# zyhbili/Dual-Space-NeRF

Hardware: AMD Instinct MI355X
Metric: rendered rays/sec (64 samples/ray), 512x512 frame (higher is better)
Workload: dtype split-f16x3 (3 x v_mfma_f32_32x32x16_f16 on hi/lo fp16 operand halves, f32 accumulate: f32-equivalent accuracy - parity bars of the tests: 1e-4 absolute on RGB / acc / weights against the reference; sigma 1e-4 absolute where |sigma| <= 100 and 4e-6 RELATIVE to max|sigma| above (this checkpoint: |sig

## Files before the change

### dual-space-nerf_amd/csrc/dsn_field16.hip

```cpp
#include "dsn_common.h"
#include "dsn_kernels.h"

typedef float f32x16 __attribute__((ext_vector_type(16)));
typedef _Float16 half8 __attribute__((ext_vector_type(8)));
#define MFMA16(a, b, c) __builtin_amdgcn_mfma_f32_32x32x16_f16((a), (b), (c), 0, 0, 0)

#if !defined(DSN_EXPERIMENTS) && (defined(F16_ABL) || defined(F16_SABL) || defined(F16_TIMING) || defined(F16_TRAIN_ABL))
#error "F16_ABL / F16_SABL / F16_TIMING are experiment switches (wrong results / debug counters): build with -DDSN_EXPERIMENTS"
#endif
#ifndef F16_SINCOS_OCML
#define F16_SINCOS_OCML 0
#endif
#ifndef F16_FENCE
#define F16_FENCE 0
#endif
#ifndef F16_SGB
#define F16_SGB 1
#endif
#ifndef F16_SGB_VALU
#define F16_SGB_VALU 4
#endif
#ifndef F16_SGB_DS
#define F16_SGB_DS 0
#endif
// ... 52 lines not shown
    char* ring;
    unsigned ring_off;
    int wave;
    int nchunk = F16_NCHUNK;
    bool spread = F16_DMA_SPREAD != 0;
    half8 h0, l0, h1, l1;
};

#ifndef F16_POS_OFFS
#define F16_POS_OFFS 0
#endif
__device__ __forceinline__ void w16_stage(const W16& w, int c) {
    const char* src = w.g + (size_t)c * 32768;
    const unsigned dst = w.ring_off + (c & 1) * 32768 + w.wave * 8192 + 4096;
#if F16_POS_OFFS
    asm volatile("s_mov_b32 m0, %1\n\ts_nop 0\n\t"
                 "global_load_lds_dwordx4 %0, off\n\tglobal_load_lds_dwordx4 %0, off offset:1024\n\t"
                 "global_load_lds_dwordx4 %0, off offset:2048\n\tglobal_load_lds_dwordx4 %0, off offset:3072"
                 : : "v"(src - 4096), "s"(dst - 4096) : "memory", "m0");
    asm volatile("s_mov_b32 m0, %1\n\ts_nop 0\n\t"
                 "global_load_lds_dwordx4 %0, off\n\tglobal_load_lds_dwordx4 %0, off offset:1024\n\t"
                 "global_load_lds_dwordx4 %0, off offset:2048\n\tglobal_load_lds_dwordx4 %0, off offset:3072"
                 : : "v"(src), "s"(dst) : "memory", "m0");
    return;
#endif
    asm volatile("s_mov_b32 m0, %1\n\ts_nop 0\n\t"
                 "global_load_lds_dwordx4 %0, off offset:-4096\n\tglobal_load_lds_dwordx4 %0, off offset:-3072\n\t"
                 "global_load_lds_dwordx4 %0, off offset:-2048\n\tglobal_load_lds_dwordx4 %0, off offset:-1024\n\t"
                 "global_load_lds_dwordx4 %0, off\n\tglobal_load_lds_dwordx4 %0, off offset:1024\n\t"
                 "global_load_lds_dwordx4 %0, off offset:2048\n\tglobal_load_lds_dwordx4 %0, off offset:3072"
                 : : "v"(src), "s"(dst) : "memory", "m0");
}
template <int I>
__device__ __forceinline__ void w16_stage_part(const W16& w, int c) {
    const char* src = w.g + (size_t)c * 32768;
    const unsigned dst = w.ring_off + (c & 1) * 32768 + w.wave * 8192 + 4096;
#if F16_POS_OFFS
    {
        const int back = I < 2 ? 4096 : 0;
        asm volatile("s_mov_b32 m0, %1\n\ts_nop 0\n\t"
                     "global_load_lds_dwordx4 %0, off offset:%2\n\tglobal_load_lds_dwordx4 %0, off offset:%3"
                     : : "v"(src - back), "s"(dst - back), "n"(2048 * (I & 1)), "n"(2048 * (I & 1) + 1024) : "memory", "m0");
        return;
    }
#endif
    asm volatile("s_mov_b32 m0, %1\n\ts_nop 0\n\t"
                 "global_load_lds_dwordx4 %0, off offset:%2\n\tglobal_load_lds_dwordx4 %0, off offset:%3"
                 : : "v"(src), "s"(dst), "n"(-4096 + 2048 * I), "n"(-3072 + 2048 * I) : "memory", "m0");
}
__device__ __forceinline__ void w16_boundary(const W16& w, int b) {
#if !(F16_ABL & 2)
    asm volatile("s_waitcnt vmcnt(0)" ::: "memory");
#endif
#if !(F16_ABL & 1)
    __syncthreads();
#endif
    const int c = b / F16_CHUNK;
#if !(F16_ABL & 4)
    if (!w.spread && c + 1 < w.nchunk) w16_stage(w, c + 1);
#endif
}
__device__ __forceinline__ void w16_read(const W16& w, int b, int lane, half8& h0, half8& l0, half8& h1, half8& l1) {
    const char* s = w.ring + ((b >> 3) & 1) * 32768 + (b & 7) * 1024 + lane * 16;
    h0 = *reinterpret_cast<const half8*>(s);
    l0 = *reinterpret_cast<const half8*>(s + 8192);
    h1 = *reinterpret_cast<const half8*>(s + 16384);
    l1 = *reinterpret_cast<const half8*>(s + 24576);
}
__device__ __forceinline__ void w16_begin_issue(W16& w, int first_blk) { w16_stage(w, first_blk / F16_CHUNK); }
__device__ __forceinline__ void w16_begin_wait(W16& w, int lane, int first_blk) {
    w16_boundary(w, first_blk);
#if !(F16_ABL & 4)
    if (w.spread && first_blk / F16_CHUNK + 1 < w.nchunk) w16_stage_part<0>(w, first_blk / F16_CHUNK + 1);
#endif
    w16_read(w, first_blk, lane, w.h0, w.l0, w.h1, w.l1);
}
__device__ __forceinline__ void w16_begin(W16& w, int lane, int first_blk) {
    w16_begin_issue(w, first_blk);
    w16_begin_wait(w, lane, first_blk);
}

struct NoHook { __device__ __forceinline__ void operator()(int) const {} };

template <int KB, bool XLS, class Hook = NoHook>
__device__ __forceinline__ void dense16(W16& w, int& blk, int lane, const half8 (&xh)[KB][2], const half8 (&xl)[KB][2],
                                        f32x16& accM, f32x16& accC, Hook&& hook = NoHook()) {
#pragma unroll
    for (int kb = 0; kb < KB; ++kb) {
#if F16_PREFETCH
        half8 n0 = w.h0, m0 = w.l0, n1 = w.h1, m1 = w.l1;
        if (blk + 1 < DSN_STREAM_BLOCKS) {
            if (((blk + 1) & (F16_CHUNK - 1)) == 0) w16_boundary(w, blk + 1);
#if !(F16_ABL & 4)
            if (w.spread) {
                const int pos = (blk + 1) & (F16_CHUNK - 1), cn = (blk + 1) / F16_CHUNK + 1;
                if (cn < w.nchunk) {
                    if (pos == 0) w16_stage_part<0>(w, cn);
                    if (pos == 1) w16_stage_part<1>(w, cn);
                    if (pos == 2) w16_stage_part<2>(w, cn);
                    if (pos == 3) w16_stage_part<3>(w, cn);
                }
            }
#endif
            w16_read(w, blk + 1, lane, n0, m0, n1, m1);
        }
#else
        if (blk > 0) {
            if ((blk & (F16_CHUNK - 1)) == 0) w16_boundary(w, blk);
            w16_read(w, blk, lane, w.h0, w.l0, w.h1, w.l1);
        }
#endif
        if (XLS) {
            accM = MFMA16(w.h0, xh[kb][0], accM);
            accC = MFMA16(w.h0, xl[kb][0], accC);
            accC = MFMA16(w.l0, xh[kb][0], accC);
            accM = MFMA16(w.h1, xh[kb][1], accM);
            accC = MFMA16(w.h1, xl[kb][1], accC);
            accC = MFMA16(w.l1, xh[kb][1], accC);
        } else {
            accM = MFMA16(w.h0, xh[kb][0], accM);
            accC = MFMA16(w.l0, xh[kb][0], accC);
            accM = MFMA16(w.h0, xl[kb][0], accM);
            accC = MFMA16(w.h1, xh[kb][1], accC);
            accM = MFMA16(w.l1, xh[kb][1], accM);
            accC = MFMA16(w.h1, xl[kb][1], accC);
        }
#if !(F16_ABL & 8)
        hook(kb);
#endif
#if F16_PREFETCH
        w.h0 = n0; w.l0 = m0; w.h1 = n1; w.l1 = m1;
#endif
        ++blk;
#if F16_SGB
#if F16_SGB_DS == 2
        __builtin_amdgcn_sched_group_barrier(0x100, 4, 0);
#endif
#pragma unroll
        for (int i = 0; i < 6; ++i) {
            __builtin_amdgcn_sched_group_barrier(0x008, 1, 0);
#if F16_SGB_DS == 1
            if (i < 4) __builtin_amdgcn_sched_group_barrier(0x100, 1, 0);
#endif
            __builtin_amdgcn_sched_group_barrier(0x002, F16_SGB_VALU, 0);
        }
        __builtin_amdgcn_sched_barrier(0);
#endif
#if F16_FENCE
        __builtin_amdgcn_sched_barrier(0);
#endif
    }
}

__device__ __forceinline__ f32x16 rows16(const float* __restrict__ v, int m, int half) {
    f32x16 o;
#pragma unroll
    for (int q = 0; q < 4; ++q) {
        const float4 t = *reinterpret_cast<const float4*>(v + 32 * m + 8 * q + 4 * half);
        o[4 * q + 0] = t.x; o[4 * q + 1] = t.y; o[4 * q + 2] = t.z; o[4 * q + 3] = t.w;
    }
    return o;
}
__device__ __forceinline__ f32x16 zero16() {
    f32x16 z;
#pragma unroll
    for (int r = 0; r < 16; ++r) z[r] = 0.0f;
    return z;
}
template <bool SCALED>
__device__ __forceinline__ void split16(const f32x16& v, half8 (&h)[2], half8 (&l)[2]) {
#pragma unroll
    for (int r = 0; r < 16; ++r) {
        const _Float16 hi = (_Float16)v[r];
        const float res = fmaf((float)hi, -1.0f, v[r]);
        h[r >> 3][r & 7] = hi;
        l[r >> 3][r & 7] = SCALED ? (_Float16)(res * DSN_LO_SCALE) : (_Float16)res;
    }
}
#define F16_FWD_SCALE 64.0f
#define F16_FWD_INV 0.015625f
__device__ __forceinline__ f32x16 unscale16(const f32x16& m, const f32x16& c) {
    f32x16 v;
#pragma unroll
    for (int r = 0; r < 16; ++r) v[r] = (m[r] + c[r]) * F16_FWD_INV;
    return v;
}
__device__ __forceinline__ f32x16 fold16(const f32x16& m, const f32x16& c) {
    f32x16 v;
#pragma unroll
    for (int r = 0; r < 16; ++r) v[r] = fmaf(c[r], DSN_LO_INV, m[r]);
    return v;
}
__device__ __forceinline__ uint32_t dsn_push_sign(uint32_t word, float v) {
    return __builtin_amdgcn_alignbit(word, __float_as_uint(v), 31);
}
__device__ __forceinline__ uint32_t dsn_active_word(uint32_t signs) { return ~signs & 0xffffu; }
#ifndef F16_KEEP_ASM
#define F16_KEEP_ASM 1
#endif
__device__ __forceinline__ float dsn_keep_active(float v, uint32_t word, int r) {
#if F16_KEEP_ASM
    uint32_t m;
    asm("v_bfe_i32 %0, %1, %2, 1" : "=v"(m) : "v"(word), "s"(15 - r));
    return __uint_as_float(__float_as_uint(v) & m);
#else
    return __uint_as_float(__float_as_uint(v) & (uint32_t)__builtin_amdgcn_sbfe((int)word, 15 - r, 1));
#endif
}
__device__ __forceinline__ uint32_t relu_bits16(f32x16& a) {
    uint32_t s = 0;
#pragma unroll
    for (int r = 0; r < 16; ++r) {
        s = dsn_push_sign(s, a[r]);
        a[r] = fmaxf(a[r], 0.0f);
    }
    return dsn_active_word(s);
}
__device__ __forceinline__ void mask16(f32x16& a, uint32_t m) {
#pragma unroll
    for (int r = 0; r < 16; ++r) a[r] = dsn_keep_active(a[r], m, r);
}

__device__ __forceinline__ void track16(float& ovf, const f32x16& v) {
#pragma unroll
    for (int r = 0; r < 16; r += 2) asm("v_max3_f32 %0, %0, |%1|, |%2|" : "+v"(ovf) : "v"(v[r]), "v"(v[r + 1]));
}
__device__ __forceinline__ float dsn_nan_flag() { return __uint_as_float(0x7fc00000u); }
// ... 60 lines not shown
            const float s0 = vv[0] * DSN_LO_SCALE, s1 = vv[1] * DSN_LO_SCALE;
            asm("v_fma_mixlo_f16 %0, %1, %2, %3 op_sel_hi:[1,0,0]" : "=v"(L) : "v"(H), "s"(k), "v"(s0));
            asm("v_fma_mixhi_f16 %0, %1, %2, %3 op_sel:[1,0,0] op_sel_hi:[1,0,0]" : "+v"(L) : "v"(H), "s"(k), "v"(s1));
        }
        typedef uint32_t u32x4 __attribute__((ext_vector_type(4)));
        u32x4 th = __builtin_bit_cast(u32x4, yh[r >> 3]), tl = __builtin_bit_cast(u32x4, yl[r >> 3]);
        th[(r & 7) >> 1] = H;
        tl[(r & 7) >> 1] = L;
        yh[r >> 3] = __builtin_bit_cast(half8, th);
        yl[r >> 3] = __builtin_bit_cast(half8, tl);
    }
#endif
    if (FWD) asm("v_max3_f32 %0, %0, %1, %2" : "+v"(ovf) : "v"(vv[0]), "v"(vv[1]));
    else asm("v_max3_f32 %0, %0, |%1|, |%2|" : "+v"(ovf) : "v"(vv[0]), "v"(vv[1]));
#if defined(DSN_EXPERIMENTS) && defined(F16_TRAIN_ABL) && (F16_TRAIN_ABL & 256)
    if (ST && kb == 7) {
        float o[16];
#pragma unroll
        for (int r = 0; r < 16; ++r) {
            float v = FWD ? (pM[r] + pC[r]) * F16_FWD_INV : fmaf(pC[r], DSN_LO_INV, pM[r]);
            v = FWD ? fmaxf(v, 0.0f) : dsn_keep_active(v, mword, r);
            o[r] = v * stscale;
        }
        store16_lines_emul(st, o);
        return;
    }
#endif
    if (ST && kb == 7 && st) {
#pragma unroll
        for (int q = 0; q < 4; ++q) {
            float o[4];
#pragma unroll
            for (int e = 0; e < 4; ++e) {
                const int r = 4 * q + e;
                float v = FWD ? (pM[r] + pC[r]) * F16_FWD_INV : fmaf(pC[r], DSN_LO_INV, pM[r]);
                v = FWD ? fmaxf(v, 0.0f) : dsn_keep_active(v, mword, r);
                o[e] = v * stscale;
            }
            *reinterpret_cast<float4*>(st + 8 * q) = make_float4(o[0], o[1], o[2], o[3]);
        }
    }
}
#ifndef F16_NT_STORE
#define F16_NT_STORE 0
#endif
typedef float f32x4 __attribute__((ext_vector_type(4)));
__device__ __forceinline__ void store16(float* st, const f32x16& v, float stscale) {
#if defined(DSN_EXPERIMENTS) && defined(F16_TRAIN_ABL) && (F16_TRAIN_ABL & 4)
    {
        const int lane = threadIdx.x & 63, hf = lane >> 5, i = lane & 3;
        const unsigned long long me = (unsigned long long)(uintptr_t)st;
#pragma unroll
        for (int j = 0; j < 4; ++j) {
            const int src = (lane & ~3) | j;
            const unsigned lo = __shfl((unsigned)me, src), hi = __shfl((unsigned)(me >> 32), src);
            float* pj = reinterpret_cast<float*>((uintptr_t)(((unsigned long long)hi << 32) | lo));
            if (pj) *reinterpret_cast<float4*>(pj - 4 * hf + 16 * hf + 4 * i) =
                make_float4(v[4 * j] * stscale, v[4 * j + 1] * stscale, v[4 * j + 2] * stscale, v[4 * j + 3] * stscale);
        }
        return;
    }
#endif
#if defined(DSN_EXPERIMENTS) && defined(F16_TRAIN_ABL) && (F16_TRAIN_ABL & 256)
    {
        float o[16];
#pragma unroll
        for (int r = 0; r < 16; ++r) o[r] = v[r] * stscale;
        store16_lines_emul(st, o);
        return;
    }
#endif
    if (!st) return;
#pragma unroll
    for (int q = 0; q < 4; ++q) {
#if F16_NT_STORE
        const f32x4 x = {v[4 * q] * stscale, v[4 * q + 1] * stscale, v[4 * q + 2] * stscale, v[4 * q + 3] * stscale};
        __builtin_nontemporal_store(x, reinterpret_cast<f32x4*>(st + 8 * q));
#else
        *reinterpret_cast<float4*>(st + 8 * q) = make_float4(v[4 * q] * stscale, v[4 * q + 1] * stscale, v[4 * q + 2] * stscale, v[4 * q + 3] * stscale);
#endif
    }
}

template <bool ST = false, bool EXTRA = false, bool HEAD = false>
__device__ __forceinline__ void layer16_fwd(W16& w, int& blk, int lane, const float* __restrict__ bias,
                                            const half8 (&xh)[8][2], const half8 (&xl)[8][2], half8 (&yh)[8][2],
                                            half8 (&yl)[8][2], uint32_t (&mk)[4], float& ovf, float* st = nullptr,
                                            const half8 (*s_pe)[F16_THREADS] = nullptr, const float* wden = nullptr, float* sg = nullptr) {
    const int half = lane >> 5;
    const int tid = threadIdx.x;
    f32x16 pM = zero16(), pC = zero16();
#if F16_BIAS_AHEAD
    f32x16 bnext = rows16(bias, 0, half);
#endif
#pragma unroll
    for (int m = 0; m < 8; ++m) {
#if F16_BIAS_AHEAD
        f32x16 aM = bnext, aC = zero16();
        if (m + 1 < 8) bnext = rows16(bias, m + 1, half);
#else
        f32x16 aM = rows16(bias, m, half), aC = zero16();
#endif
        uint32_t bits = 0;
        if (m == 0) dense16<8, false>(w, blk, lane, xh, xl, aM, aC);
        else dense16<8, false>(w, blk, lane, xh, xl, aM, aC, [&](int kb) {
            epi_slice<true, ST, HEAD>(pM, pC, kb, 0u, bits, yh[m - 1], yl[m - 1], ovf, (ST && st) ? st + F16_ST_M(m - 1) : nullptr, 1.0f,
                                      HEAD ? wden + 32 * (m - 1) + 4 * half : nullptr, sg); });
        if (EXTRA) {
            half8 qh[2][2], ql[2][2];
            qh[0][0] = s_pe[0][tid]; qh[0][1] = s_pe[1][tid]; qh[1][0] = s_pe[2][tid]; qh[1][1] = s_pe[3][tid];
            ql[0][0] = s_pe[4][tid]; ql[0][1] = s_pe[5][tid]; ql[1][0] = s_pe[6][tid]; ql[1][1] = s_pe[7][tid];
            dense16<2, false>(w, blk, lane, qh, ql, aM, aC);
        }
        if (m > 0) { if ((m - 1) & 1) mk[(m - 1) >> 1] |= dsn_active_word(bits) << 16; else mk[(m - 1) >> 1] = dsn_active_word(bits); }
        pM = aM; pC = aC;
    }
    {
        uint32_t bits = 0;
#pragma unroll
        for (int kb = 0; kb < 8; ++kb)
            epi_slice<true, ST, HEAD>(pM, pC, kb, 0u, bits, yh[7], yl[7], ovf, (ST && st) ? st + F16_ST_M(7) : nullptr, 1.0f,
                                      HEAD ? wden + 32 * 7 + 4 * half : nullptr, sg);
        mk[3] |= dsn_active_word(bits) << 16;
    }
}
template <bool ST = false>
__device__ __forceinline__ void layer16_bwd(W16& w, int& blk, int lane, const half8 (&xh)[8][2],
                                            const half8 (&xl)[8][2], half8 (&yh)[8][2], half8 (&yl)[8][2],
                                            const uint32_t (&mk)[4], float& ovf, float* st = nullptr, float stscale = F16_GUNSCALE) {
    f32x16 pM = zero16(), pC = zero16();
    uint32_t dummy = 0;
#pragma unroll
    for (int m = 0; m < 8; ++m) {
        f32x16 aM = zero16(), aC = zero16();
        const uint32_t mw = m > 0 ? ((mk[(m - 1) >> 1] >> (16 * ((m - 1) & 1))) & 0xffffu) : 0u;
        if (m == 0) dense16<8, true>(w, blk, lane, xh, xl, aM, aC);
        else dense16<8, true>(w, blk, lane, xh, xl, aM, aC, [&](int kb) { epi_slice<false, ST>(pM, pC, kb, mw, dummy, yh[m - 1], yl[m - 1], ovf, (ST && st) ? st + F16_ST_M(m - 1) : nullptr, stscale); });
        pM = aM; pC = aC;
    }
    const uint32_t mw = (mk[3] >> 16) & 0xffffu;
#pragma unroll
    for (int kb = 0; kb < 8; ++kb) epi_slice<false, ST>(pM, pC, kb, mw, dummy, yh[7], yl[7], ovf, (ST && st) ? st + F16_ST_M(7) : nullptr, stscale);
}

#define F16_FULL 0
#define F16_FWD 1
#define F16_BWD 2
#define F16_TRAIN 3
#define F16_DEN 4
#define F16_FIRST_BWD_BLOCK (OFF_L6T / DSN_BLK)
#define F16_DEN_BLOCKS (F16_FIRST_BWD_BLOCK - 4 * 8)
static_assert(F16_DEN_BLOCKS % F16_CHUNK == 0, "the density-only kernel streams whole chunks");
template <int MODE>
__global__ void __launch_bounds__(F16_THREADS, 1)
k_field16(const float* __restrict__ packed, const DsnFrameState* __restrict__ fs, const float* __restrict__ x_c,
          int64_t N, const int32_t* __restrict__ active_list, const int32_t* __restrict__ active_count,
          float* __restrict__ sigma, float* __restrict__ essence, float* __restrict__ grad,
          uint4* __restrict__ masks, int32_t* __restrict__ pos_list, int32_t* __restrict__ pos_count,
          float* __restrict__ tr_h, float* __restrict__ tr_a, float* __restrict__ tr_rr, int64_t slot_base, int64_t rec_cap,
          const int32_t* __restrict__ sel, int32_t* __restrict__ flag_count) {
    constexpr bool ST = MODE == F16_TRAIN;
    __shared__ __attribute__((aligned(16))) char ring[F16_RING_SLOTS * 4096];
    __shared__ uint32_t s_mask[7][4][F16_THREADS];
    __shared__ __attribute__((aligned(16))) float s_vec[256 + 2304 + 8];
    __shared__ __attribute__((aligned(16))) half8 s_pe[8][F16_THREADS];
    __shared__ int s_app[8];
#ifndef F16_SHARE_SIMD
    DSN_OWN_SIMD();
#endif
    const int tid0 = threadIdx.x;
    const int lane0 = threadIdx.x & 63;
    const int wave = __builtin_amdgcn_readfirstlane(threadIdx.x >> 6);
    int64_t count = (active_list ? (int64_t)(*active_count) : N) - slot_base;
    if (MODE == F16_BWD && count > rec_cap) count = rec_cap;
    const int64_t ntiles = (count + 127) / 128;
    if ((int64_t)blockIdx.x >= ntiles) return;
    for (int i = tid0; i < 256 + 2304 + 8; i += F16_THREADS)
        s_vec[i] = i < 256 ? fs->bias0[i] : (i < 2560 ? packed[OFF_B1 + (i - 256)] : packed[OFF_SCAL + (i - 2560)]);
    for (int i = tid0; i < 256 + (OFF_WDEN - OFF_B1); i += F16_THREADS) s_vec[i] *= F16_FWD_SCALE;
    const float* const v_bias0 = s_vec;
    const float* const v_b1 = s_vec + 256;
    const float* const v_brgb1 = s_vec + 256 + (OFF_BRGB1 - OFF_B1);
    const float* const v_wden = s_vec + 256 + (OFF_WDEN - OFF_B1);
    const float* const v_wrgb3 = s_vec + 256 + (OFF_WRGB3 - OFF_B1);
    const float* const v_scal = s_vec + 2560;
    W16 w;
    w.g = reinterpret_cast<const char*>(packed + OFF16_BASE) + wave * 8192 + 4096 + lane0 * 16;
    w.ring = ring;
    w.ring_off = (unsigned)(uintptr_t)(__attribute__((address_space(3))) char*)ring;
    w.wave = wave;
    if (MODE == F16_FWD) w.nchunk = F16_FIRST_BWD_BLOCK / F16_CHUNK;
    if (MODE == F16_DEN) w.nchunk = F16_DEN_BLOCKS / F16_CHUNK;
    if (MODE == F16_TRAIN) w.spread = false;
    auto tile_point = [&](int64_t t, bool& ok, int64_t& ls) -> int64_t {
        int64_t sl = (t * 4 + wave) * 32 + (lane0 & 31);
        ok = sl < count;
        if (!ok) sl = count - 1;
        ls = sel ? (int64_t)sel[sl] : slot_base + sl;
        return active_list ? (int64_t)active_list[ls] : ls;
    };
    bool valid_n;
    int64_t lslot_n;
    int64_t pt_n = tile_point(blockIdx.x, valid_n, lslot_n);
    float xn[3] = {x_c[3 * pt_n], x_c[3 * pt_n + 1], x_c[3 * pt_n + 2]};
  for (int64_t tile = blockIdx.x; tile < ntiles; tile += gridDim.x) {
    int tid = tid0, lane = lane0;
    asm volatile("" : "+v"(tid), "+v"(lane), "+v"(w.g));
    const int half = lane >> 5;
#if F16_TIMING
    unsigned long long tstamp[6], rstamp[6];
#endif
    F16_STAMP(0);
    w16_begin_issue(w, MODE == F16_BWD ? F16_FIRST_BWD_BLOCK : 0);
#if !F16_NEXT_POINT
    if (tile != (int64_t)blockIdx.x) { pt_n = tile_point(tile, valid_n, lslot_n); xn[0] = x_c[3 * pt_n]; xn[1] = x_c[3 * pt_n + 1]; xn[2] = x_c[3 * pt_n + 2]; }
#endif
    const bool valid = valid_n;
    const int64_t lslot = lslot_n, pt = pt_n;
    const float xa[3] = {xn[0], xn[1], xn[2]};
    const bool more = F16_NEXT_POINT && MODE != F16_TRAIN && tile + gridDim.x < ntiles;
    if (more) pt_n = tile_point(tile + gridDim.x, valid_n, lslot_n);
#define NEXT_POINT() do { if (more) { xn[0] = x_c[3 * pt_n]; xn[1] = x_c[3 * pt_n + 1]; xn[2] = x_c[3 * pt_n + 2]; } } while (0)
    w16_begin_wait(w, lane, MODE == F16_BWD ? F16_FIRST_BWD_BLOCK : 0);
    int blk = MODE == F16_BWD ? F16_FIRST_BWD_BLOCK : 0;
    F16_STAMP(1);

#define MK_STORE(L, mk) { if (MODE != F16_DEN) { s_mask[L][0][tid] = mk[0]; s_mask[L][1][tid] = mk[1]; s_mask[L][2][tid] = mk[2]; s_mask[L][3][tid] = mk[3]; } }
#define MK_LOAD(L, mk) { mk[0] = s_mask[L][0][tid]; mk[1] = s_mask[L][1][tid]; mk[2] = s_mask[L][2][tid]; mk[3] = s_mask[L][3][tid]; }
    uint32_t mk[4];
    half8 ah[8][2], al[8][2], bh[8][2], bl[8][2];
    float ovf = packed[DSN_SPLIT_UNSAFE_FIELD];
    uint4* mrec = masks ? masks + ((size_t)(MODE == F16_BWD ? lslot : pt) * 2 + half) * 7 : nullptr;
    const int64_t tr_ls = N * 256;
#if defined(DSN_EXPERIMENTS) && defined(F16_TRAIN_ABL)
    const int64_t pt_st = (F16_TRAIN_ABL & 8) ? (pt & 4095) : ((F16_TRAIN_ABL & 16) ? (pt & 255) : pt);
    const int64_t sl_st = (tile * 4 + wave) * 32 + (lane & 31);
    const int64_t row_off = (F16_TRAIN_ABL & 32) ? (sl_st >> 5) * 8192 + (sl_st & 31) * 32 : pt_st * 256;
    float* const th = ST && valid && !(F16_TRAIN_ABL & 1) ? tr_h + row_off + 4 * half : nullptr;
    float* const ta = ST && valid && !(F16_TRAIN_ABL & 2) ? tr_a + row_off + 4 * half : nullptr;
#else
    float* const th = ST && valid ? tr_h + pt * 256 + 4 * half : nullptr;
    float* const ta = ST && valid ? tr_a + pt * 256 + 4 * half : nullptr;
#endif

  if (MODE != F16_BWD) {
    half8 ph[2][2], pl[2][2];
    {
        f32x16 pe[2];
#pragma unroll
        for (int t = 0; t < 30; ++t) {
            float s, c;
#if F16_SINCOS_OCML
            sincosf(xa[t % 3] * (float)(1 << (t / 3)), &s, &c);
#else
            dsn_sincos(xa[t % 3] * (float)(1 << (t / 3)), s, c);
#endif
            pe[t >> 4][t & 15] = half ? c : s;
        }
        pe[1][14] = half ? xa[1] : xa[0];
        pe[1][15] = half ? 0.0f : xa[2];
        split16<false>(pe[0], ph[0], pl[0]);
        split16<false>(pe[1], ph[1], pl[1]);
        s_pe[0][tid] = ph[0][0]; s_pe[1][tid] = ph[0][1]; s_pe[2][tid] = ph[1][0]; s_pe[3][tid] = ph[1][1];
        s_pe[4][tid] = pl[0][0]; s_pe[5][tid] = pl[0][1]; s_pe[6][tid] = pl[1][0]; s_pe[7][tid] = pl[1][1];
    }

    F16_STAMP(2);
#pragma unroll
    for (int m = 0; m < 8; ++m) {
        f32x16 aM = rows16(v_bias0, m, half), aC = zero16();
        dense16<2, false>(w, blk, lane, ph, pl, aM, aC);
        f32x16 v = unscale16(aM, aC);
        const uint32_t bits = relu_bits16(v);
        if (m & 1) mk[m >> 1] |= bits << 16; else mk[m >> 1] = bits;
        if (ST) store16(th ? th + 0 * tr_ls + F16_ST_M(m) : nullptr, v, 1.0f);
        track16(ovf, v);
        split16<false>(v, ah[m], al[m]);
    }
    MK_STORE(0, mk)
    layer16_fwd<ST>(w, blk, lane, v_b1 + 0 * 256, ah, al, bh, bl, mk, ovf, th ? th + 1 * tr_ls : nullptr); MK_STORE(1, mk)
    NEXT_POINT();
    layer16_fwd<ST>(w, blk, lane, v_b1 + 1 * 256, bh, bl, ah, al, mk, ovf, th ? th + 2 * tr_ls : nullptr); MK_STORE(2, mk)
    layer16_fwd<ST>(w, blk, lane, v_b1 + 2 * 256, ah, al, bh, bl, mk, ovf, th ? th + 3 * tr_ls : nullptr); MK_STORE(3, mk)
#if F16_PIPE_LATE
    layer16_fwd<ST, true, false>(w, blk, lane, v_b1 + 3 * 256, bh, bl, ah, al, mk, ovf, th ? th + 4 * tr_ls : nullptr, s_pe);
    MK_STORE(4, mk)
    layer16_fwd<ST>(w, blk, lane, v_b1 + 4 * 256, ah, al, bh, bl, mk, ovf, th ? th + 5 * tr_ls : nullptr); MK_STORE(5, mk)
    float sg_part = 0.0f;
    layer16_fwd<ST, false, true>(w, blk, lane, v_b1 + 5 * 256, bh, bl, ah, al, mk, ovf, th ? th + 6 * tr_ls : nullptr, nullptr, v_wden,
                                 &sg_part);
#else
#pragma unroll
    for (int m = 0; m < 8; ++m) {
        f32x16 aM = rows16(v_b1 + 3 * 256, m, half), aC = zero16();
        dense16<8, false>(w, blk, lane, bh, bl, aM, aC);
        {
            half8 qh[2][2], ql[2][2];
            qh[0][0] = s_pe[0][tid]; qh[0][1] = s_pe[1][tid]; qh[1][0] = s_pe[2][tid]; qh[1][1] = s_pe[3][tid];
            ql[0][0] = s_pe[4][tid]; ql[0][1] = s_pe[5][tid]; ql[1][0] = s_pe[6][tid]; ql[1][1] = s_pe[7][tid];
            dense16<2, false>(w, blk, lane, qh, ql, aM, aC);
        }
        f32x16 v = unscale16(aM, aC);
        const uint32_t bits = relu_bits16(v);
        if (m & 1) mk[m >> 1] |= bits << 16; else mk[m >> 1] = bits;
        if (ST) store16(th ? th + 4 * tr_ls + F16_ST_M(m) : nullptr, v, 1.0f);
        track16(ovf, v);
        split16<false>(v, ah[m], al[m]);
    }
    MK_STORE(4, mk)
    layer16_fwd<ST>(w, blk, lane, v_b1 + 4 * 256, ah, al, bh, bl, mk, ovf, th ? th + 5 * tr_ls : nullptr); MK_STORE(5, mk)
    float sg_part = 0.0f;
#pragma unroll
    for (int m = 0; m < 8; ++m) {
        f32x16 aM = rows16(v_b1 + 5 * 256, m, half), aC = zero16();
        dense16<8, false>(w, blk, lane, bh, bl, aM, aC);
        f32x16 v = unscale16(aM, aC);
        const uint32_t bits = relu_bits16(v);
        if (m & 1) mk[m >> 1] |= bits << 16; else mk[m >> 1] = bits;
        if (ST) store16(th ? th + 6 * tr_ls + F16_ST_M(m) : nullptr, v, 1.0f);
        const f32x16 wd = rows16(v_wden, m, half);
#pragma unroll
        for (int r = 0; r < 16; ++r) sg_part = fmaf(wd[r], v[r], sg_part);
        track16(ovf, v);
        split16<false>(v, ah[m], al[m]);
    }
#endif
    F16_STAMP(3);
    sg_part += __shfl_xor(sg_part, 32);
    const float sg = sg_part + v_scal[0];
    const bool flag_fwd = !(fmaxf(ovf, __shfl_xor(ovf, 32)) < F16_RANGE);
    if (valid && half == 0) sigma[pt] = flag_fwd ? dsn_nan_flag() : sg;
    if (MODE != F16_TRAIN && flag_fwd && valid && half == 0 && flag_count) atomicAdd(flag_count, 1);
    ovf = flag_fwd ? __builtin_inff() : 0.0f;
    if (MODE == F16_DEN) { __syncthreads(); continue; }
    bool write_rec = ST && valid;
    if (MODE == F16_FWD) {
        const bool pos = valid && half == 0 && (sg > 0.0f || flag_fwd);
        const unsigned long long bm = __ballot(pos);
        const int cnt = __popcll(bm);
        if (lane == 0) s_app[wave] = cnt;
        __syncthreads();
        if (tid == 0) {
            const int tot = s_app[0] + s_app[1] + s_app[2] + s_app[3];
            s_app[4] = tot ? atomicAdd(pos_count, tot) : 0;
        }
        __syncthreads();
        int base = s_app[4];
        for (int k = 0; k < wave; ++k) base += s_app[k];
        const int my = base + __popcll(bm & ((1ull << lane) - 1ull));
        if (pos) pos_list[my] = (int32_t)pt;
        const int rslot = __shfl(my, lane & 31);
        write_rec = ((bm >> (lane & 31)) & 1ull) != 0 && (int64_t)rslot < rec_cap;
        mrec = masks + ((size_t)rslot * 2 + half) * 7;
    }
    if (MODE == F16_FWD || MODE == F16_TRAIN) {
        MK_STORE(6, mk)
        if (write_rec) {
#pragma unroll
            for (int L = 0; L < 7; ++L)
                mrec[L] = make_uint4(s_mask[L][0][tid], s_mask[L][1][tid], s_mask[L][2][tid], s_mask[L][3][tid]);
        }
    }
    {
        float e0 = 0.f, e1 = 0.f, e2 = 0.f;
#pragma unroll
        for (int m = 0; m < 4; ++m) {
            f32x16 aM = rows16(v_brgb1, m, half), aC = zero16();
            dense16<8, false>(w, blk, lane, ah, al, aM, aC);
            const f32x16 v = unscale16(aM, aC);
            const f32x16 w0 = rows16(v_wrgb3 + 0 * 128, m, half);
            const f32x16 w1 = rows16(v_wrgb3 + 1 * 128, m, half);
            const f32x16 w2 = rows16(v_wrgb3 + 2 * 128, m, half);
            if (ST && valid) {
                f32x16 xr;
#pragma unroll
                for (int r = 0; r < 16; ++r) xr[r] = fmaxf(v[r], 0.0f);
                store16(tr_rr + pt * 128 + 4 * half + 32 * m, xr, 1.0f);
            }
#pragma unroll
            for (int r = 0; r < 16; ++r) {
                const float x = fmaxf(v[r], 0.0f);
                e0 = fmaf(w0[r], x, e0); e1 = fmaf(w1[r], x, e1); e2 = fmaf(w2[r], x, e2);
            }
        }
        e0 += __shfl_xor(e0, 32); e1 += __shfl_xor(e1, 32); e2 += __shfl_xor(e2, 32);
        if (valid && half == 0) {
            essence[3 * pt + 0] = e0 + v_scal[1];
            essence[3 * pt + 1] = e1 + v_scal[2];
            essence[3 * pt + 2] = e2 + v_scal[3];
        }
    }

#if F16_TIMING
    F16_STAMP(4);
    if (MODE == F16_FWD && tid == 0) {
        for (int i = 0; i < 4; ++i) { atomicAdd(&g_f16_timing[i], tstamp[i + 1] - tstamp[i]); atomicAdd(&g_f16_timing[8 + i], rstamp[i + 1] - rstamp[i]); }
        atomicAdd(&g_f16_timing[7], 1ull);
    }
#endif
    if (MODE == F16_FWD) { __syncthreads(); continue; }
  } else {
#pragma unroll
    for (int L = 0; L < 7; ++L) {
        const uint4 q = mrec[L];
        s_mask[L][0][tid] = q.x; s_mask[L][1][tid] = q.y; s_mask[L][2][tid] = q.z; s_mask[L][3][tid] = q.w;
    }
    MK_LOAD(6, mk)
  }

#pragma unroll
    for (int m = 0; m < 8; ++m) {
        f32x16 g = rows16(v_wden, m, half);
#pragma unroll
        for (int r = 0; r < 16; ++r) g[r] *= F16_GSCALE;
        mask16(g, (mk[m >> 1] >> (16 * (m & 1))) & 0xffffu);
        if (ST) store16(ta ? ta + 6 * tr_ls + F16_ST_M(m) : nullptr, g, F16_GUNSCALE);
        split16<true>(g, ah[m], al[m]);
    }
    MK_LOAD(5, mk) layer16_bwd<ST>(w, blk, lane, ah, al, bh, bl, mk, ovf, ta ? ta + 5 * tr_ls : nullptr);
    if (MODE == F16_BWD) NEXT_POINT();
    MK_LOAD(4, mk) layer16_bwd<ST>(w, blk, lane, bh, bl, ah, al, mk, ovf, ta ? ta + 4 * tr_ls : nullptr);
    MK_LOAD(3, mk)
    f32x16 dpe[2];
#pragma unroll
    for (int m = 0; m < 8; ++m) {
        f32x16 aM = zero16(), aC = zero16();
        dense16<8, true>(w, blk, lane, ah, al, aM, aC);
        f32x16 v = fold16(aM, aC);
        mask16(v, (mk[m >> 1] >> (16 * (m & 1))) & 0xffffu);
        if (ST) store16(ta ? ta + 3 * tr_ls + F16_ST_M(m) : nullptr, v, F16_GUNSCALE);
        track16(ovf, v);
        split16<true>(v, bh[m], bl[m]);
    }
#pragma unroll
    for (int b = 0; b < 2; ++b) {
        f32x16 aM = zero16(), aC = zero16();
        dense16<8, true>(w, blk, lane, ah, al, aM, aC);
        dpe[b] = fold16(aM, aC);
    }
    MK_LOAD(2, mk) layer16_bwd<ST>(w, blk, lane, bh, bl, ah, al, mk, ovf, ta ? ta + 2 * tr_ls : nullptr);
    MK_LOAD(1, mk) layer16_bwd<ST>(w, blk, lane, ah, al, bh, bl, mk, ovf, ta ? ta + 1 * tr_ls : nullptr);
    MK_LOAD(0, mk) layer16_bwd<ST>(w, blk, lane, bh, bl, ah, al, mk, ovf, ta ? ta + 0 * tr_ls : nullptr);
#pragma unroll
    for (int b = 0; b < 2; ++b) {
        f32x16 aM = zero16(), aC = zero16();
        dense16<8, true>(w, blk, lane, ah, al, aM, aC);
        const f32x16 v = fold16(aM, aC);
#pragma unroll
        for (int r = 0; r < 16; ++r) dpe[b][r] += v[r];
    }

    {
        float xb[3] = {xa[0], xa[1], xa[2]};
        asm volatile("" : "+v"(xb[0]), "+v"(xb[1]), "+v"(xb[2]));
        float g[3] = {0.f, 0.f, 0.f};
#pragma unroll
        for (int t = 0; t < 30; ++t) {
            const int j = t / 3, a = t % 3;
            float s, c;
#if F16_SINCOS_OCML
            sincosf(xb[a] * (float)(1 << j), &s, &c);
#else
            dsn_sincos(xb[a] * (float)(1 << j), s, c);
#endif
            const float d = dpe[t >> 4][t & 15];
            const float term = (d * (half ? s : c)) * (float)(1 << j);
            g[a] += half ? -term : term;
        }
        const float i30 = dpe[1][14], i31 = dpe[1][15];
        if (half) g[1] += i30; else { g[0] += i30; g[2] += i31; }
        g[0] += __shfl_xor(g[0], 32); g[1] += __shfl_xor(g[1], 32); g[2] += __shfl_xor(g[2], 32);
        if (valid && half == 0) {
            grad[3 * pt] = g[0] * F16_GUNSCALE; grad[3 * pt + 1] = g[1] * F16_GUNSCALE; grad[3 * pt + 2] = g[2] * F16_GUNSCALE;
        }
    }
    const bool flagged = !(fmaxf(ovf, __shfl_xor(ovf, 32)) < F16_RANGE_SCALED);
    if (flagged && valid && half == 0) {
        if (MODE == F16_TRAIN) { if (pos_count) atomicAdd(pos_count, 1); }
        else { sigma[pt] = dsn_nan_flag(); if (flag_count) atomicAdd(flag_count, 1); }
    }
    if (MODE == F16_TRAIN) break;
    __syncthreads();
  }
}

void dsn_launch_field16(const float* packed, const DsnFrameState* fs, const float* x_c, int64_t N,
                        const int32_t* active_list, const int32_t* active_count, float* sigma, float* essence,
                        float* grad, hipStream_t st, int32_t* flag_count) {
    int64_t blocks = (N + 127) / 128;
    if (blocks == 0) return;
    hipLaunchKernelGGL(k_field16<F16_FULL>, dim3((unsigned)std::min<int64_t>(blocks, dsn_cu_count())), dim3(F16_THREADS), 0, st, packed, fs, x_c, N,
                       active_list, active_count, sigma, essence, grad, (uint4*)nullptr, (int32_t*)nullptr,
                       (int32_t*)nullptr, (float*)nullptr, (float*)nullptr, (float*)nullptr, (int64_t)0, (int64_t)0, (const int32_t*)nullptr,
                       flag_count);
}
void dsn_launch_field16_from(const float* packed, const DsnFrameState* fs, const float* x_c, int64_t N, const int32_t* list,
                             const int32_t* count, int64_t slot_base, float* sigma, float* essence, float* grad, hipStream_t st,
                             int32_t* flag_count) {
    int64_t blocks = (N - slot_base + 127) / 128;
    if (blocks <= 0) return;
    hipLaunchKernelGGL(k_field16<F16_FULL>, dim3((unsigned)std::min<int64_t>(blocks, dsn_cu_count())), dim3(F16_THREADS), 0, st, packed, fs, x_c, N, list, count, sigma,
                       essence, grad, (uint4*)nullptr, (int32_t*)nullptr, (int32_t*)nullptr, (float*)nullptr, (float*)nullptr,
                       (float*)nullptr, slot_base, (int64_t)0, (const int32_t*)nullptr, flag_count);
}
void dsn_launch_field16_train(const float* packed, const DsnFrameState* fs, const float* x_c, int64_t N, float* sigma,
                              float* essence, float* grad, float* tr_h, float* tr_a, float* tr_rr, void* masks, hipStream_t st,
                              int32_t* range_count, const int32_t* row_list, const int32_t* row_count) {
    int64_t blocks = (N + 127) / 128;
    if (blocks == 0) return;
    hipLaunchKernelGGL(k_field16<F16_TRAIN>, dim3((unsigned)blocks), dim3(F16_THREADS), 0, st, packed, fs, x_c, N,
                       row_list, row_count, sigma, essence, grad, (uint4*)masks, (int32_t*)nullptr,
                       range_count, tr_h, tr_a, tr_rr, (int64_t)0, N, (const int32_t*)nullptr, (int32_t*)nullptr);
}
void dsn_launch_field16_fwd(const float* packed, const DsnFrameState* fs, const float* x_c, int64_t N,
                            const int32_t* active_list, const int32_t* active_count, float* sigma, float* essence,
                            void* masks, int32_t* pos_list, int32_t* pos_count, hipStream_t st, int64_t rec_cap, int32_t* flag_count) {
    int64_t blocks = (N + 127) / 128;
    if (blocks == 0) return;
    hipLaunchKernelGGL(k_field16<F16_FWD>, dim3((unsigned)std::min<int64_t>(blocks, dsn_cu_count())), dim3(F16_THREADS), 0, st, packed, fs, x_c, N,
                       active_list, active_count, sigma, essence, (float*)nullptr, (uint4*)masks, pos_list, pos_count,
                       (float*)nullptr, (float*)nullptr, (float*)nullptr, (int64_t)0, rec_cap, (const int32_t*)nullptr, flag_count);
}
void dsn_launch_field16_den(const float* packed, const DsnFrameState* fs, const float* x_c, int64_t N,
                            const int32_t* active_list, const int32_t* active_count, float* sigma, hipStream_t st,
                            int32_t* flag_count) {
    int64_t blocks = (N + 127) / 128;
    if (blocks == 0) return;
    hipLaunchKernelGGL(k_field16<F16_DEN>, dim3((unsigned)std::min<int64_t>(blocks, dsn_cu_count())), dim3(F16_THREADS), 0, st, packed, fs, x_c, N,
                       active_list, active_count, sigma, (float*)nullptr, (float*)nullptr, (uint4*)nullptr, (int32_t*)nullptr,
// ... 1330 lines not shown
```

Baseline: 27.87 million.

## Carry each layer's final output-slice epilogue into the next layer's first MFMA block

New measurement: 28.31 million, median of 6. 1.6% higher.

```diff
diff --git a/dual-space-nerf_amd/csrc/dsn_field16.hip b/dual-space-nerf_amd/csrc/dsn_field16.hip
--- a/dual-space-nerf_amd/csrc/dsn_field16.hip
+++ b/dual-space-nerf_amd/csrc/dsn_field16.hip
@@ -158,7 +158,7 @@
 
 struct NoHook { __device__ __forceinline__ void operator()(int) const {} };
 
-template <int KB, bool XLS, class Hook = NoHook>
+template <int KB, bool XLS, int VALU = F16_SGB_VALU, class Hook = NoHook>
 __device__ __forceinline__ void dense16(W16& w, int& blk, int lane, const half8 (&xh)[KB][2], const half8 (&xl)[KB][2],
                                         f32x16& accM, f32x16& accC, Hook&& hook = NoHook()) {
 #pragma unroll
@@ -218,7 +218,7 @@
 #if F16_SGB_DS == 1
             if (i < 4) __builtin_amdgcn_sched_group_barrier(0x100, 1, 0);
 #endif
-            __builtin_amdgcn_sched_group_barrier(0x002, F16_SGB_VALU, 0);
+            __builtin_amdgcn_sched_group_barrier(0x002, VALU, 0);
         }
         __builtin_amdgcn_sched_barrier(0);
 #endif
@@ -445,11 +445,51 @@
     }
 }
 
-template <bool ST = false, bool EXTRA = false, bool HEAD = false>
+struct Pend16 {
+    f32x16 M, C;
+    uint32_t bits;
+    uint32_t w3;
+};
+#define F16_CARRY_VALU 5
+#define F16_CARRY_FIRST(kb) ((kb) < 5 ? (kb) - 1 : 2 * (kb) - 6)
+#define F16_CARRY_LAST(kb) ((kb) < 5 ? (kb) - 1 : 2 * (kb) - 5)
+__device__ __forceinline__ void pend_slice(const Pend16& p, int s, f32x16& tM, f32x16& tC) {
+    float m0 = p.M[2 * s], m1 = p.M[2 * s + 1], c0 = p.C[2 * s], c1 = p.C[2 * s + 1];
+    asm("" : "+v"(m0), "+v"(m1), "+v"(c0), "+v"(c1));
+    tM[2 * s] = m0; tM[2 * s + 1] = m1; tC[2 * s] = c0; tC[2 * s + 1] = c1;
+}
+template <bool HEAD = false>
+__device__ __forceinline__ void carry_fwd(Pend16& p, int kb, half8 (&yh)[2], half8 (&yl)[2], float& ovf, uint32_t* mdst,
+                                          const float* wd = nullptr, float* sg = nullptr) {
+    if (kb < 1 || kb > 6) return;
+#pragma unroll
+    for (int s = F16_CARRY_FIRST(kb); s <= F16_CARRY_LAST(kb); ++s) {
+        f32x16 tM, tC;
+        pend_slice(p, s, tM, tC);
+        epi_slice<true, false, HEAD>(tM, tC, s, 0u, p.bits, yh, yl, ovf, nullptr, 1.0f, wd, sg);
+    }
+    if (kb == 6) {
+        p.w3 |= dsn_active_word(p.bits) << 16;
+        if (mdst) *mdst = p.w3;
+    }
+}
+__device__ __forceinline__ void carry_bwd(Pend16& p, int kb, half8 (&yh)[2], half8 (&yl)[2], float& ovf) {
+    if (kb < 1 || kb > 6) return;
+    uint32_t dummy = 0;
+#pragma unroll
+    for (int s = F16_CARRY_FIRST(kb); s <= F16_CARRY_LAST(kb); ++s) {
+        f32x16 tM, tC;
+        pend_slice(p, s, tM, tC);
+        epi_slice<false, false>(tM, tC, s, p.w3, dummy, yh, yl, ovf);
+    }
+}
+
+template <bool ST = false, bool EXTRA = false, bool HEAD = false, bool CIN = false, bool COUT = false>
 __device__ __forceinline__ void layer16_fwd(W16& w, int& blk, int lane, const float* __restrict__ bias,
-                                            const half8 (&xh)[8][2], const half8 (&xl)[8][2], half8 (&yh)[8][2],
+                                            half8 (&xh)[8][2], half8 (&xl)[8][2], half8 (&yh)[8][2],
                                             half8 (&yl)[8][2], uint32_t (&mk)[4], float& ovf, float* st = nullptr,
-                                            const half8 (*s_pe)[F16_THREADS] = nullptr, const float* wden = nullptr, float* sg = nullptr) {
+                                            const half8 (*s_pe)[F16_THREADS] = nullptr, const float* wden = nullptr, float* sg = nullptr,
+                                            Pend16* pd = nullptr, uint32_t* mdst = nullptr) {
     const int half = lane >> 5;
     const int tid = threadIdx.x;
     f32x16 pM = zero16(), pC = zero16();
@@ -465,7 +505,8 @@
         f32x16 aM = rows16(bias, m, half), aC = zero16();
 #endif
         uint32_t bits = 0;
-        if (m == 0) dense16<8, false>(w, blk, lane, xh, xl, aM, aC);
+        if (m == 0 && CIN) dense16<8, false, F16_CARRY_VALU>(w, blk, lane, xh, xl, aM, aC, [&](int kb) { carry_fwd(*pd, kb, xh[7], xl[7], ovf, mdst); });
+        else if (m == 0) dense16<8, false>(w, blk, lane, xh, xl, aM, aC);
         else dense16<8, false>(w, blk, lane, xh, xl, aM, aC, [&](int kb) {
             epi_slice<true, ST, HEAD>(pM, pC, kb, 0u, bits, yh[m - 1], yl[m - 1], ovf, (ST && st) ? st + F16_ST_M(m - 1) : nullptr, 1.0f,
                                       HEAD ? wden + 32 * (m - 1) + 4 * half : nullptr, sg); });
@@ -478,7 +519,9 @@
         if (m > 0) { if ((m - 1) & 1) mk[(m - 1) >> 1] |= dsn_active_word(bits) << 16; else mk[(m - 1) >> 1] = dsn_active_word(bits); }
         pM = aM; pC = aC;
     }
-    {
+    if (COUT) {
+        pd->M = pM; pd->C = pC; pd->bits = 0; pd->w3 = mk[3];
+    } else {
         uint32_t bits = 0;
 #pragma unroll
         for (int kb = 0; kb < 8; ++kb)
@@ -487,21 +530,32 @@
         mk[3] |= dsn_active_word(bits) << 16;
     }
 }
-template <bool ST = false>
-__device__ __forceinline__ void layer16_bwd(W16& w, int& blk, int lane, const half8 (&xh)[8][2],
-                                            const half8 (&xl)[8][2], half8 (&yh)[8][2], half8 (&yl)[8][2],
-                                            const uint32_t (&mk)[4], float& ovf, float* st = nullptr, float stscale = F16_GUNSCALE) {
+template <bool EXTRA = false, bool HEAD = false, bool COUT = true>
+__device__ __forceinline__ void layer16_fwd_carry(W16& w, int& blk, int lane, const float* __restrict__ bias, half8 (&xh)[8][2],
+                                                  half8 (&xl)[8][2], half8 (&yh)[8][2], half8 (&yl)[8][2], uint32_t (&mk)[4],
+                                                  float& ovf, Pend16& pd, uint32_t* mdst,
+                                                  const half8 (*s_pe)[F16_THREADS] = nullptr, const float* wden = nullptr,
+                                                  float* sg = nullptr) {
+    layer16_fwd<false, EXTRA, HEAD, true, COUT>(w, blk, lane, bias, xh, xl, yh, yl, mk, ovf, nullptr, s_pe, wden, sg, &pd, mdst);
+}
+template <bool ST = false, bool CIN = false, bool COUT = false>
+__device__ __forceinline__ void layer16_bwd(W16& w, int& blk, int lane, half8 (&xh)[8][2],
+                                            half8 (&xl)[8][2], half8 (&yh)[8][2], half8 (&yl)[8][2],
+                                            const uint32_t (&mk)[4], float& ovf, float* st = nullptr, float stscale = F16_GUNSCALE,
+                                            Pend16* pd = nullptr) {
     f32x16 pM = zero16(), pC = zero16();
     uint32_t dummy = 0;
 #pragma unroll
     for (int m = 0; m < 8; ++m) {
         f32x16 aM = zero16(), aC = zero16();
         const uint32_t mw = m > 0 ? ((mk[(m - 1) >> 1] >> (16 * ((m - 1) & 1))) & 0xffffu) : 0u;
-        if (m == 0) dense16<8, true>(w, blk, lane, xh, xl, aM, aC);
+        if (m == 0 && CIN) dense16<8, true, F16_CARRY_VALU>(w, blk, lane, xh, xl, aM, aC, [&](int kb) { carry_bwd(*pd, kb, xh[7], xl[7], ovf); });
+        else if (m == 0) dense16<8, true>(w, blk, lane, xh, xl, aM, aC);
         else dense16<8, true>(w, blk, lane, xh, xl, aM, aC, [&](int kb) { epi_slice<false, ST>(pM, pC, kb, mw, dummy, yh[m - 1], yl[m - 1], ovf, (ST && st) ? st + F16_ST_M(m - 1) : nullptr, stscale); });
         pM = aM; pC = aC;
     }
     const uint32_t mw = (mk[3] >> 16) & 0xffffu;
+    if (COUT) { pd->M = pM; pd->C = pC; pd->bits = 0; pd->w3 = mw; return; }
 #pragma unroll
     for (int kb = 0; kb < 8; ++kb) epi_slice<false, ST>(pM, pC, kb, mw, dummy, yh[7], yl[7], ovf, (ST && st) ? st + F16_ST_M(7) : nullptr, stscale);
 }
@@ -511,6 +565,7 @@
 #define F16_BWD 2
 #define F16_TRAIN 3
 #define F16_DEN 4
+#define F16_CARRY_MODE(M) ((M) == F16_FWD || (M) == F16_BWD || (M) == F16_DEN || (M) == F16_FULL)
 #define F16_FIRST_BWD_BLOCK (OFF_L6T / DSN_BLK)
 #define F16_DEN_BLOCKS (F16_FIRST_BWD_BLOCK - 4 * 8)
 static_assert(F16_DEN_BLOCKS % F16_CHUNK == 0, "the density-only kernel streams whole chunks");
@@ -523,6 +578,7 @@
           float* __restrict__ tr_h, float* __restrict__ tr_a, float* __restrict__ tr_rr, int64_t slot_base, int64_t rec_cap,
           const int32_t* __restrict__ sel, int32_t* __restrict__ flag_count) {
     constexpr bool ST = MODE == F16_TRAIN;
+    constexpr bool CARRY = F16_PIPE_LATE && F16_CARRY_MODE(MODE);
     __shared__ __attribute__((aligned(16))) char ring[F16_RING_SLOTS * 4096];
     __shared__ uint32_t s_mask[7][4][F16_THREADS];
     __shared__ __attribute__((aligned(16))) float s_vec[256 + 2304 + 8];
@@ -589,6 +645,8 @@
     F16_STAMP(1);
 
 #define MK_STORE(L, mk) { if (MODE != F16_DEN) { s_mask[L][0][tid] = mk[0]; s_mask[L][1][tid] = mk[1]; s_mask[L][2][tid] = mk[2]; s_mask[L][3][tid] = mk[3]; } }
+#define MK_STORE_C(L, mk) { if (MODE != F16_DEN) { s_mask[L][0][tid] = mk[0]; s_mask[L][1][tid] = mk[1]; s_mask[L][2][tid] = mk[2]; } }
+#define MK_WORD3(L) (MODE != F16_DEN ? &s_mask[L][3][tid] : nullptr)
 #define MK_LOAD(L, mk) { mk[0] = s_mask[L][0][tid]; mk[1] = s_mask[L][1][tid]; mk[2] = s_mask[L][2][tid]; mk[3] = s_mask[L][3][tid]; }
     uint32_t mk[4];
     half8 ah[8][2], al[8][2], bh[8][2], bl[8][2];
@@ -629,6 +687,39 @@
     }
 
     F16_STAMP(2);
+    Pend16 pd;
+    float sg_part = 0.0f;
+  if (CARRY) {
+    {
+        f32x16 pM = zero16(), pC = zero16();
+#pragma unroll
+        for (int m = 0; m < 8; ++m) {
+            f32x16 aM = rows16(v_bias0, m, half), aC = zero16();
+            uint32_t bits = 0;
+            if (m == 0) dense16<2, false>(w, blk, lane, ph, pl, aM, aC);
+            else dense16<2, false, 6>(w, blk, lane, ph, pl, aM, aC, [&](int kb) {
+#pragma unroll
+                for (int s = 0; s < 4; ++s) epi_slice<true>(pM, pC, 4 * kb + s, 0u, bits, ah[m - 1], al[m - 1], ovf); });
+            if (m > 0) { if ((m - 1) & 1) mk[(m - 1) >> 1] |= dsn_active_word(bits) << 16; else mk[(m - 1) >> 1] = dsn_active_word(bits); }
+            pM = aM; pC = aC;
+        }
+        pd.M = pM; pd.C = pC; pd.bits = 0; pd.w3 = mk[3];
+    }
+    MK_STORE_C(0, mk)
+    layer16_fwd_carry(w, blk, lane, v_b1 + 0 * 256, ah, al, bh, bl, mk, ovf, pd, MK_WORD3(0));
+    MK_STORE_C(1, mk)
+    NEXT_POINT();
+    layer16_fwd_carry(w, blk, lane, v_b1 + 1 * 256, bh, bl, ah, al, mk, ovf, pd, MK_WORD3(1));
+    MK_STORE_C(2, mk)
+    layer16_fwd_carry(w, blk, lane, v_b1 + 2 * 256, ah, al, bh, bl, mk, ovf, pd, MK_WORD3(2));
+    MK_STORE_C(3, mk)
+    layer16_fwd_carry<true>(w, blk, lane, v_b1 + 3 * 256, bh, bl, ah, al, mk, ovf, pd, MK_WORD3(3), s_pe);
+    MK_STORE_C(4, mk)
+    layer16_fwd_carry(w, blk, lane, v_b1 + 4 * 256, ah, al, bh, bl, mk, ovf, pd, MK_WORD3(4));
+    MK_STORE_C(5, mk)
+    layer16_fwd_carry<false, true, MODE != F16_DEN>(w, blk, lane, v_b1 + 5 * 256, bh, bl, ah, al, mk, ovf, pd, MK_WORD3(5), nullptr, v_wden,
+                                                    &sg_part);
+  } else {
 #pragma unroll
     for (int m = 0; m < 8; ++m) {
         f32x16 aM = rows16(v_bias0, m, half), aC = zero16();
@@ -649,7 +740,6 @@
     layer16_fwd<ST, true, false>(w, blk, lane, v_b1 + 3 * 256, bh, bl, ah, al, mk, ovf, th ? th + 4 * tr_ls : nullptr, s_pe);
     MK_STORE(4, mk)
     layer16_fwd<ST>(w, blk, lane, v_b1 + 4 * 256, ah, al, bh, bl, mk, ovf, th ? th + 5 * tr_ls : nullptr); MK_STORE(5, mk)
-    float sg_part = 0.0f;
     layer16_fwd<ST, false, true>(w, blk, lane, v_b1 + 5 * 256, bh, bl, ah, al, mk, ovf, th ? th + 6 * tr_ls : nullptr, nullptr, v_wden,
                                  &sg_part);
 #else
@@ -672,7 +762,6 @@
     }
     MK_STORE(4, mk)
     layer16_fwd<ST>(w, blk, lane, v_b1 + 4 * 256, ah, al, bh, bl, mk, ovf, th ? th + 5 * tr_ls : nullptr); MK_STORE(5, mk)
-    float sg_part = 0.0f;
 #pragma unroll
     for (int m = 0; m < 8; ++m) {
         f32x16 aM = rows16(v_b1 + 5 * 256, m, half), aC = zero16();
@@ -688,6 +777,8 @@
         split16<false>(v, ah[m], al[m]);
     }
 #endif
+  }
+    auto trunk_done = [&]() {
     F16_STAMP(3);
     sg_part += __shfl_xor(sg_part, 32);
     const float sg = sg_part + v_scal[0];
@@ -695,7 +786,7 @@
     if (valid && half == 0) sigma[pt] = flag_fwd ? dsn_nan_flag() : sg;
     if (MODE != F16_TRAIN && flag_fwd && valid && half == 0 && flag_count) atomicAdd(flag_count, 1);
     ovf = flag_fwd ? __builtin_inff() : 0.0f;
-    if (MODE == F16_DEN) { __syncthreads(); continue; }
+    if (MODE == F16_DEN) return;
     bool write_rec = ST && valid;
     if (MODE == F16_FWD) {
         const bool pos = valid && half == 0 && (sg > 0.0f || flag_fwd);
@@ -724,8 +815,40 @@
                 mrec[L] = make_uint4(s_mask[L][0][tid], s_mask[L][1][tid], s_mask[L][2][tid], s_mask[L][3][tid]);
         }
     }
+    };
+    constexpr bool CARRY_HEAD = CARRY && MODE != F16_DEN;
+    if (!CARRY_HEAD) trunk_done();
+    if (MODE == F16_DEN) { __syncthreads(); continue; }
     {
         float e0 = 0.f, e1 = 0.f, e2 = 0.f;
+      if (CARRY_HEAD) {
+        f32x16 pM = zero16(), pC = zero16(), w0 = zero16(), w1 = zero16(), w2 = zero16();
+        auto rgb_slice = [&](int kb) {
+#pragma unroll
+            for (int e = 0; e < 2; ++e) {
+                const int r = 2 * kb + e;
+                const float x = fmaxf((pM[r] + pC[r]) * F16_FWD_INV, 0.0f);
+                e0 = fmaf(w0[r], x, e0); e1 = fmaf(w1[r], x, e1); e2 = fmaf(w2[r], x, e2);
+            }
+            asm volatile("" : "+v"(e0), "+v"(e1), "+v"(e2));
+        };
+#pragma unroll
+        for (int m = 0; m < 4; ++m) {
+            f32x16 aM = rows16(v_brgb1, m, half), aC = zero16();
+            if (m == 0) {
+                dense16<8, false, F16_CARRY_VALU>(w, blk, lane, ah, al, aM, aC, [&](int kb) {
+                    carry_fwd<true>(pd, kb, ah[7], al[7], ovf, nullptr, v_wden + 32 * 7 + 4 * half, &sg_part); });
+                mk[3] = pd.w3;
+                trunk_done();
+            } else {
+                dense16<8, false>(w, blk, lane, ah, al, aM, aC, rgb_slice);
+            }
+            pM = aM; pC = aC;
+            w0 = rows16(v_wrgb3 + 0 * 128, m, half); w1 = rows16(v_wrgb3 + 1 * 128, m, half); w2 = rows16(v_wrgb3 + 2 * 128, m, half);
+        }
+#pragma unroll
+        for (int kb = 0; kb < 8; ++kb) rgb_slice(kb);
+      } else {
 #pragma unroll
         for (int m = 0; m < 4; ++m) {
             f32x16 aM = rows16(v_brgb1, m, half), aC = zero16();
@@ -746,6 +869,7 @@
                 e0 = fmaf(w0[r], x, e0); e1 = fmaf(w1[r], x, e1); e2 = fmaf(w2[r], x, e2);
             }
         }
+      }
         e0 += __shfl_xor(e0, 32); e1 += __shfl_xor(e1, 32); e2 += __shfl_xor(e2, 32);
         if (valid && half == 0) {
             essence[3 * pt + 0] = e0 + v_scal[1];
@@ -780,11 +904,27 @@
         if (ST) store16(ta ? ta + 6 * tr_ls + F16_ST_M(m) : nullptr, g, F16_GUNSCALE);
         split16<true>(g, ah[m], al[m]);
     }
-    MK_LOAD(5, mk) layer16_bwd<ST>(w, blk, lane, ah, al, bh, bl, mk, ovf, ta ? ta + 5 * tr_ls : nullptr);
+    Pend16 rd;
+    MK_LOAD(5, mk) layer16_bwd<ST, false, CARRY>(w, blk, lane, ah, al, bh, bl, mk, ovf, ta ? ta + 5 * tr_ls : nullptr, F16_GUNSCALE, &rd);
     if (MODE == F16_BWD) NEXT_POINT();
-    MK_LOAD(4, mk) layer16_bwd<ST>(w, blk, lane, bh, bl, ah, al, mk, ovf, ta ? ta + 4 * tr_ls : nullptr);
+    MK_LOAD(4, mk) layer16_bwd<ST, CARRY, CARRY>(w, blk, lane, bh, bl, ah, al, mk, ovf, ta ? ta + 4 * tr_ls : nullptr, F16_GUNSCALE, &rd);
     MK_LOAD(3, mk)
     f32x16 dpe[2];
+  if (CARRY) {
+    f32x16 pM = zero16(), pC = zero16();
+    uint32_t dummy = 0;
+#pragma unroll
+    for (int m = 0; m < 10; ++m) {
+        f32x16 aM = zero16(), aC = zero16();
+        const uint32_t mw = (m > 0 && m <= 8) ? ((mk[(m - 1) >> 1] >> (16 * ((m - 1) & 1))) & 0xffffu) : 0u;
+        if (m == 0) dense16<8, true, F16_CARRY_VALU>(w, blk, lane, ah, al, aM, aC, [&](int kb) { carry_bwd(rd, kb, ah[7], al[7], ovf); });
+        else if (m <= 8) dense16<8, true>(w, blk, lane, ah, al, aM, aC, [&](int kb) { epi_slice<false>(pM, pC, kb, mw, dummy, bh[(m - 1) & 7], bl[(m - 1) & 7], ovf); });
+        else dense16<8, true>(w, blk, lane, ah, al, aM, aC, [&](int kb) {
+            dpe[0][2 * kb] = fmaf(pC[2 * kb], DSN_LO_INV, pM[2 * kb]); dpe[0][2 * kb + 1] = fmaf(pC[2 * kb + 1], DSN_LO_INV, pM[2 * kb + 1]); });
+        pM = aM; pC = aC;
+    }
+    dpe[1] = fold16(pM, pC);
+  } else {
 #pragma unroll
     for (int m = 0; m < 8; ++m) {
         f32x16 aM = zero16(), aC = zero16();
@@ -801,13 +941,15 @@
         dense16<8, true>(w, blk, lane, ah, al, aM, aC);
         dpe[b] = fold16(aM, aC);
     }
-    MK_LOAD(2, mk) layer16_bwd<ST>(w, blk, lane, bh, bl, ah, al, mk, ovf, ta ? ta + 2 * tr_ls : nullptr);
-    MK_LOAD(1, mk) layer16_bwd<ST>(w, blk, lane, ah, al, bh, bl, mk, ovf, ta ? ta + 1 * tr_ls : nullptr);
-    MK_LOAD(0, mk) layer16_bwd<ST>(w, blk, lane, bh, bl, ah, al, mk, ovf, ta ? ta + 0 * tr_ls : nullptr);
+  }
+    MK_LOAD(2, mk) layer16_bwd<ST, false, CARRY>(w, blk, lane, bh, bl, ah, al, mk, ovf, ta ? ta + 2 * tr_ls : nullptr, F16_GUNSCALE, &rd);
+    MK_LOAD(1, mk) layer16_bwd<ST, CARRY, CARRY>(w, blk, lane, ah, al, bh, bl, mk, ovf, ta ? ta + 1 * tr_ls : nullptr, F16_GUNSCALE, &rd);
+    MK_LOAD(0, mk) layer16_bwd<ST, CARRY, CARRY>(w, blk, lane, bh, bl, ah, al, mk, ovf, ta ? ta + 0 * tr_ls : nullptr, F16_GUNSCALE, &rd);
 #pragma unroll
     for (int b = 0; b < 2; ++b) {
         f32x16 aM = zero16(), aC = zero16();
-        dense16<8, true>(w, blk, lane, ah, al, aM, aC);
+        if (CARRY && b == 0) dense16<8, true, F16_CARRY_VALU>(w, blk, lane, ah, al, aM, aC, [&](int kb) { carry_bwd(rd, kb, ah[7], al[7], ovf); });
+        else dense16<8, true>(w, blk, lane, ah, al, aM, aC);
         const f32x16 v = fold16(aM, aC);
 #pragma unroll
         for (int r = 0; r < 16; ++r) dpe[b][r] += v[r];
```
